# ndoll1998/lightgrad

Measured on AMD Instinct MI355X. Metric: mnist_mlp_train_steps_per_sec_batch1024_per_gpu, higher is better.
Workload: dtype f32; 1 GPU; mnist_mlp_784x512x10_bias_batch1024_mse_adabelief_lr1e-3 (fwd+bwd+allreduce+optimizer); batch_per_gpu=1024, global_batch=1024, parallelism=dp1, optimizer_kernel=fused, input_requires_grad=True, dispatch=hipGraph replay (python tape captured once; 13 consecutive steps per graph), steps_per_graph=13, device=AMD Instinct (gfx950), compute_units=256, clock_mhz=2400

## Files before the change

### lightgrad_amd/csrc/gemm.hip

```cpp
#include "common.h"
#include "gelu_common.h"
#include "adam_common.h"
#include "tail_jobs.h"
#include "mse_finalize.h"
#include "head_fwd_body.h"
#include <cstdlib>
#include <cstring>
#include <type_traits>

namespace lg {

typedef float f32x16 __attribute__((ext_vector_type(16)));
typedef unsigned int u32x4 __attribute__((ext_vector_type(4)));
typedef float f32x4 __attribute__((ext_vector_type(4)));

#ifndef LG_SMALL_PD
#define LG_SMALL_PD 2
#endif
constexpr int kSmallTilePrefetch = LG_SMALL_PD;
#ifndef LG_WAVE_PRIVATE_PD
#define LG_WAVE_PRIVATE_PD 1
#endif
constexpr int kWavePrivatePrefetch = LG_WAVE_PRIVATE_PD;

struct FastDiv {
    uint32_t m, s;
    __device__ __forceinline__ int div(int n) const { return int((uint64_t(uint32_t(n)) * m) >> s); }
};
static FastDiv make_fastdiv(int64_t d) {
    if (d < 1) d = 1;
    uint32_t l = 0;
    while ((int64_t(1) << l) < d) ++l;
    FastDiv f;
    f.m = uint32_t((uint64_t(1) << (31 + l)) / uint64_t(d) + 1);
    f.s = 31 + l;
    return f;
}

struct GemmArgs {
    const float* A;
    const float* B;
    float*       C;
    int64_t M, N, K;
    int64_t lda, ldb, ldc;
    int64_t sA, sB, sC;
    int64_t sA2, sB2, sC2;
    int     batch_inner;
    int     tiles_m, tiles_n;
    int     nwg;
    int     accumulate;
    const float* bias;
    const float* addend;
    int64_t      ldadd;
    int     group_m;
    int     k_slices;
    int64_t k_per_slice;
    float*  W;
    int*    tickets;
    float*  rowsum;
    int     rowsum_accumulate;
    FastDiv div_per_batch, div_slices, div_gspan, div_group, div_last_group, div_batch_inner;
    int     k_tail;
    short   relu_a, relu_b;
    int     act;
    float*  aux;
    int     multi;
    int64_t boff[3], coff[3], biasoff[3];
    int     seg_k, seg_steps;
    int64_t seg_jump[2];
    const AdamPlan* adam_c;
    const AdamPlan* adam_r;
#ifdef LG_GEMM_TIMELINE
    unsigned long long* tl;
#endif
};

#ifdef LG_GEMM_TIMELINE
#define LG_TL(slot) do { if (g.tl && threadIdx.x == 0) g.tl[size_t(blockIdx.x) * 8 + (slot)] = wall_clock64(); } while (0)
#else
#define LG_TL(slot) do { } while (0)
#endif

__device__ __forceinline__ int xcd_remap(int bid, int nwg) {
    const int q = nwg >> 3, r = nwg & 7;
    const int xcd = bid & 7, pos = bid >> 3;
    const int base = xcd < r ? xcd * (q + 1) : r * (q + 1) + (xcd - r) * q;
    return base + pos;
}

template <int BM, int BN> constexpr bool kHasExtras = BM * BN < 256 * 256;
template <int BM, int BN, int KG = 1> constexpr bool kCanSplitK = kHasExtras<BM, BN> && KG == 1;
template <int BM, int BN, int KG = 1> constexpr bool kCanAdam = BM * BN <= 128 * 128 && KG == 1;

#ifdef LG_GEMM_GATHER_STAGING
template <int BM, int BN, bool XKC> constexpr bool kGatherStaging = !XKC && BM * BN == 256 * 256;
#else
template <int BM, int BN, bool XKC> constexpr bool kGatherStaging = false;
#endif
template <int BM, int BN, int WM, int WN, int KG> constexpr bool kWavePrivateTile = KG > 1 && WM * WN == 1 && BM == 32 && BN == 32;
template <int BM, int BN, int BK, bool AKC, bool BKC, int KG>
constexpr int gemm_lds_floats() {
    constexpr int BKS = BK * KG;
    constexpr bool ALK = AKC || kGatherStaging<BM, BN, AKC>, BLK = BKC || kGatherStaging<BM, BN, BKC>;
    return 2 * ((ALK ? BM * (BKS + 4) : BKS * BM) + (BLK ? BN * (BKS + 4) : BKS * BN));
}

template <int BM, int BN, int BK, int WM, int WN, bool AKC, bool BKC, bool VA, bool VB, int PD, int KG = 1, int XT = 0, bool WP = false>
__global__ void __launch_bounds__(WM * WN * KG * 64) sgemm_mfma(GemmArgs g) {
#define LG_TILE_OWNS_LDS 1
#define LG_TILE_BID blockIdx.x
#define LG_TILE_WAVE_PRIVATE WP
#include "gemm_tile_body.inc"
#undef LG_TILE_WAVE_PRIVATE
#undef LG_TILE_OWNS_LDS
#undef LG_TILE_BID
}

struct HeadChain {
    HeadFwd h;
    int*    tickets;
    int     stride;
    int     per_row;
    int*    status;
};
static const HeadChain*& pending_chain() { static const HeadChain* p = nullptr; return p; }
constexpr int kChainTicketBase = 16384, kChainTicketStride = 32, kChainRowBlocks = 64;
template <int OMAX, int PD>
__global__ void __launch_bounds__(256) sgemm_bias_head_fwd(GemmArgs g, HeadChain c) {
    constexpr int BM = 64, BN = 32, BK = 32, WM = 2, WN = 1, KG = 2, XT = 0;
    constexpr bool AKC = true, BKC = true, VA = true, VB = true;
    __shared__ __attribute__((aligned(16))) float lds[gemm_lds_floats<BM, BN, BK, AKC, BKC, KG>()];
    if (int(blockIdx.x) < g.nwg) {
        int* const signal_tickets = c.tickets;
        const int signal_stride = c.stride, signal_per_row = c.per_row;
#define LG_TILE_OWNS_LDS 0
#define LG_TILE_BID int(blockIdx.x)
#undef LG_TILE_SIGNAL
#define LG_TILE_SIGNAL 1
#include "gemm_tile_body.inc"
#undef LG_TILE_SIGNAL
#undef LG_TILE_BID
#undef LG_TILE_OWNS_LDS
    } else {
        const HeadFwd& a = c.h;
        const int tid = threadIdx.x, lane = tid & 63, wave = tid >> 6;
        const int wn = a.outs * a.hidden;
        for (int i = tid * 4; i < wn; i += 1024) *reinterpret_cast<float4*>(lds + i) = *reinterpret_cast<const float4*>(a.w + i);
        const int64_t row0 = int64_t(int(blockIdx.x) - g.nwg) * 4;
        int* const ticket = c.tickets + int(row0 / BM) * c.stride;
        const int64_t block_rows = a.rows - (row0 / BM) * BM < BM ? a.rows - (row0 / BM) * BM : BM;
        const int readers = int((block_rows + 3) / 4);
        int* const flag = ticket + 16;
        int* const done = ticket + 17;
        __shared__ int seen;
        if (tid == 0) {
            int ok = 1;
            const unsigned long long t0 = wall_clock64();
            while (__hip_atomic_load(flag, __ATOMIC_RELAXED, __HIP_MEMORY_SCOPE_AGENT) == 0) {
                __builtin_amdgcn_s_sleep(2);
                if (wall_clock64() - t0 > 200000000ull) {
                    __hip_atomic_fetch_or(c.status, LG_STATUS_HANDOFF_TIMEOUT, __ATOMIC_RELAXED, __HIP_MEMORY_SCOPE_SYSTEM);
                    ok = 0;
                    break;
                }
            }
            seen = ok;
        }
        __syncthreads();
        __builtin_amdgcn_fence(__ATOMIC_ACQUIRE, "wavefront");
        const int64_t row = row0 + wave;
        if (row < a.rows) head_fwd_row<OMAX, true>(a, lds, row, lane);
        if (tid == 0 && seen) {
            if (__hip_atomic_fetch_add(done, 1, __ATOMIC_RELAXED, __HIP_MEMORY_SCOPE_AGENT) == readers - 1) {
                __hip_atomic_store(done, 0, __ATOMIC_RELAXED, __HIP_MEMORY_SCOPE_AGENT);
                __hip_atomic_store(flag, 0, __ATOMIC_RELAXED, __HIP_MEMORY_SCOPE_AGENT);
            }
        }
    }
}

template <int PD, bool SECOND_BKC = false>
__global__ void __launch_bounds__(256) sgemm_pair_wgrad_xgrad(GemmArgs first, GemmArgs second) {
    constexpr int L1 = gemm_lds_floats<64, 64, 32, false, false, 1>(), L2 = gemm_lds_floats<64, 64, 32, true, SECOND_BKC, 1>();
    __shared__ __attribute__((aligned(16))) float lds[L1 > L2 ? L1 : L2];
    constexpr int BM = 64, BN = 64, BK = 32, WM = 2, WN = 2, KG = 1, XT = 0;
    constexpr bool VA = true, VB = true;
#define LG_TILE_OWNS_LDS 0
    if (int(blockIdx.x) < first.nwg) {
        constexpr bool AKC = false, BKC = false;
        const GemmArgs& g = first;
#define LG_TILE_BID int(blockIdx.x)
#include "gemm_tile_body.inc"
#undef LG_TILE_BID
    } else {
        constexpr bool AKC = true, BKC = SECOND_BKC;
        const GemmArgs& g = second;
#define LG_TILE_BID (int(blockIdx.x) - first.nwg)
#include "gemm_tile_body.inc"
#undef LG_TILE_BID
    }
#undef LG_TILE_OWNS_LDS
}

int lg_mse_finalize_job(const float* row_loss, int64_t rows, float inv_n, float* loss);
struct PairFirsts { GemmArgs w[2]; };
struct LossJob {
    const float* row_loss;
    float*       loss;
    int64_t      rows;
    float        inv_n;
};
template <int PD>
__global__ void __launch_bounds__(256) sgemm_triple_wgrad2_xgrad(PairFirsts firsts, GemmArgs second, LossJob job) {
    constexpr int L1 = gemm_lds_floats<64, 64, 32, false, false, 1>(), L2 = gemm_lds_floats<64, 64, 32, true, false, 1>();
    __shared__ __attribute__((aligned(16))) float lds[L1 > L2 ? L1 : L2];
    constexpr int BM = 64, BN = 64, BK = 32, WM = 2, WN = 2, KG = 1, XT = 0;
    constexpr bool VA = true, VB = true;
#define LG_TILE_OWNS_LDS 0
    const int n0w = firsts.w[0].nwg, n1w = firsts.w[1].nwg;
    if (int(blockIdx.x) < n0w + n1w) {
        constexpr bool AKC = false, BKC = false;
        const int which = int(blockIdx.x) >= n0w ? 1 : 0;
        const GemmArgs g = firsts.w[which];
#define LG_TILE_BID (int(blockIdx.x) - (which ? n0w : 0))
#include "gemm_tile_body.inc"
#undef LG_TILE_BID
    } else if (int(blockIdx.x) < n0w + n1w + second.nwg) {
        constexpr bool AKC = true, BKC = false;
        const GemmArgs& g = second;
#define LG_TILE_BID (int(blockIdx.x) - n0w - n1w)
#include "gemm_tile_body.inc"
#undef LG_TILE_BID
    } else {
        finalize_loss(job.row_loss, job.rows, job.inv_n, job.loss, lds);
    }
#undef LG_TILE_OWNS_LDS
}

constexpr int kGroupMax = 14;
struct GroupProduct {
    const float* A;
    const float* B;
    float*       C;
    float*       W;
    int*         tickets;
    float*       rowsum;
    int64_t      M, N, K, lda, ldb, ldc, k_per_slice;
    int          tiles_m, tiles_n, nwg, accumulate, group_m, k_slices, rowsum_accumulate, k_tail;
    FastDiv      div_per_batch, div_slices, div_gspan, div_group, div_last_group, div_batch_inner;
};
static GroupProduct pack_product(const GemmArgs& g) {
    return GroupProduct{g.A, g.B, g.C, g.W, g.tickets, g.rowsum, g.M, g.N, g.K, g.lda, g.ldb, g.ldc, g.k_per_slice,
                        g.tiles_m, g.tiles_n, g.nwg, g.accumulate, g.group_m, g.k_slices, g.rowsum_accumulate, g.k_tail,
                        g.div_per_batch, g.div_slices, g.div_gspan, g.div_group, g.div_last_group, g.div_batch_inner};
}
__device__ __forceinline__ GemmArgs unpack_product(const GroupProduct& p) {
    GemmArgs g{};
    g.A = p.A; g.B = p.B; g.C = p.C; g.W = p.W; g.tickets = p.tickets; g.rowsum = p.rowsum;
    g.M = p.M; g.N = p.N; g.K = p.K; g.lda = p.lda; g.ldb = p.ldb; g.ldc = p.ldc; g.k_per_slice = p.k_per_slice;
    g.tiles_m = p.tiles_m; g.tiles_n = p.tiles_n; g.nwg = p.nwg; g.accumulate = p.accumulate; g.group_m = p.group_m;
    g.k_slices = p.k_slices; g.rowsum_accumulate = p.rowsum_accumulate; g.k_tail = p.k_tail;
    g.div_per_batch = p.div_per_batch; g.div_slices = p.div_slices; g.div_gspan = p.div_gspan; g.div_group = p.div_group;
    g.div_last_group = p.div_last_group; g.div_batch_inner = p.div_batch_inner;
    g.batch_inner = 1;
    return g;
}

struct GemmGroup {
    GroupProduct p[kGroupMax];
    int      first[kGroupMax + 1];
    int      count;
    const float* cs_in;
    float*       cs_out;
    int64_t      cs_rows, cs_cols, cs_ld;
    int          cs_accumulate, cs_wgs;
    int          tail_wgs;
    TailGroup    tail;
};

static_assert(sizeof(GemmGroup) <= 4096, "the group travels as kernel arguments");

template <int PD>
__global__ void __launch_bounds__(256) sgemm_group_wgrad(GemmGroup grp) {
    __shared__ __attribute__((aligned(16))) float lds[gemm_lds_floats<64, 64, 32, false, false, 1>()];
    constexpr int BM = 64, BN = 64, BK = 32, WM = 2, WN = 2, KG = 1, XT = 0;
    constexpr bool VA = true, VB = true, AKC = false, BKC = false;
    if (int(blockIdx.x) < grp.cs_wgs) {
        const int q = threadIdx.x >> 6, cl = threadIdx.x & 63;
        const int64_t col = int64_t(blockIdx.x) * 64 + cl;
        const bool live = col < grp.cs_cols;
        const float* in = grp.cs_in + (live ? col : 0);
        float acc[8] = {0.f, 0.f, 0.f, 0.f, 0.f, 0.f, 0.f, 0.f};
        int64_t r = q;
        for (; r + 28 < grp.cs_rows; r += 32) {
#pragma unroll
            for (int e = 0; e < 8; ++e) acc[e] += in[(r + 4 * e) * grp.cs_ld];
        }
        for (; r < grp.cs_rows; r += 4) acc[0] += in[r * grp.cs_ld];
        lds[threadIdx.x] = ((acc[0] + acc[1]) + (acc[2] + acc[3])) + ((acc[4] + acc[5]) + (acc[6] + acc[7]));
        __syncthreads();
        if (q == 0 && live) {
            const float v = (lds[cl] + lds[64 + cl]) + (lds[128 + cl] + lds[192 + cl]);
            grp.cs_out[col] = grp.cs_accumulate ? grp.cs_out[col] + v : v;
        }
        return;
    }
    const int bid = int(blockIdx.x) - grp.cs_wgs;
    if (bid >= grp.first[grp.count]) {
        tail_group_body(grp.tail, bid - grp.first[grp.count]);
        return;
    }
    int which = 0;
    while (which + 1 < grp.count && bid >= grp.first[which + 1]) ++which;
    const GemmArgs g = unpack_product(grp.p[which]);
// ... 9 lines not shown
template <int BM, int BN, int BK, int WM, int WN, bool AKC, bool BKC, int KG>
static bool launch_layout(const GemmArgs& g, bool va, bool vb) {
    dim3 grid(g.nwg), block(WM * WN * KG * 64);
    hipStream_t s = rt().stream;
    constexpr int PD = (BM * BN <= 64 * 64) ? kSmallTilePrefetch : 2;
    static_assert(BM * BN < 256 * 256 || PD <= 2, "a third K-tile in flight does not fit the 256x256 tile's 128 registers: ring registers would spill while their loads are in flight");
    if constexpr (kWavePrivateTile<BM, BN, WM, WN, KG> && AKC && BKC) {
        static const char* kloop_env = getenv("LG_GEMM_KLOOP");
        if (va && vb && !(kloop_env && strcmp(kloop_env, "coop") == 0)) {
            constexpr int WPD = kWavePrivatePrefetch;
            if (g.multi) hipLaunchKernelGGL((sgemm_mfma<BM, BN, BK, WM, WN, true, true, true, true, WPD, KG, 1, true>), grid, block, 0, s, g);
            else         hipLaunchKernelGGL((sgemm_mfma<BM, BN, BK, WM, WN, true, true, true, true, WPD, KG, 0, true>), grid, block, 0, s, g);
            return true;
        }
    }
    if constexpr (kHasExtras<BM, BN>) {
        if constexpr (AKC && BKC)  { if (g.multi) { hipLaunchKernelGGL((sgemm_mfma<BM, BN, BK, WM, WN, AKC, BKC, true, true, PD, KG, 1>), grid, block, 0, s, g); return false; } }
        if constexpr (AKC && !BKC) { if (g.seg_k) { hipLaunchKernelGGL((sgemm_mfma<BM, BN, BK, WM, WN, AKC, BKC, true, true, PD, KG, 2>), grid, block, 0, s, g); return false; } }
    }
    if constexpr (!kHasExtras<BM, BN>) {
        hipLaunchKernelGGL((sgemm_mfma<BM, BN, BK, WM, WN, AKC, BKC, true, true, PD, KG>), grid, block, 0, s, g);
        return false;
    }
    if (va && vb)  hipLaunchKernelGGL((sgemm_mfma<BM, BN, BK, WM, WN, AKC, BKC, true, true, PD, KG>), grid, block, 0, s, g);
    else if (va)   hipLaunchKernelGGL((sgemm_mfma<BM, BN, BK, WM, WN, AKC, BKC, true, false, 1, KG>), grid, block, 0, s, g);
    else if (vb)   hipLaunchKernelGGL((sgemm_mfma<BM, BN, BK, WM, WN, AKC, BKC, false, true, 1, KG>), grid, block, 0, s, g);
    else           hipLaunchKernelGGL((sgemm_mfma<BM, BN, BK, WM, WN, AKC, BKC, false, false, 1, KG>), grid, block, 0, s, g);
    return false;
}

#ifdef LG_GEMM_TIMELINE
static void lg_debug_timeline_state(unsigned long long* buf, int nwg, int slices, int tiles);
#endif
struct PairState {
    int      active = 0;
    int      count = 0;
    bool     second_bkc = false;
    GemmArgs args[3];
    bool     is_s[3] = {false, false, false};
    int64_t  batch[3] = {1, 1, 1};
    int64_t  tiles = 0;
    LossJob  job{};
};
static PairState& pair_state() { static PairState p; return p; }

static void pair_launch_single(const GemmArgs& g, bool is_s) {
    dim3 grid(g.nwg), block(256);
    constexpr int PD = kSmallTilePrefetch;
    if (!is_s) hipLaunchKernelGGL((sgemm_mfma<64, 64, 32, 2, 2, false, false, true, true, PD, 1>), grid, block, 0, rt().stream, g);
    else if (pair_state().second_bkc) hipLaunchKernelGGL((sgemm_mfma<64, 64, 32, 2, 2, true, true, true, true, PD, 1>), grid, block, 0, rt().stream, g);
    else           hipLaunchKernelGGL((sgemm_mfma<64, 64, 32, 2, 2, true, false, true, true, PD, 1>), grid, block, 0, rt().stream, g);
}

static int pair_retune(GemmArgs& g, int64_t others_nwg) {
    const int64_t tiles = int64_t(g.tiles_m) * g.tiles_n;
    static const char* pair_slices_env = getenv("LG_GEMM_PAIR_SLICES");
    if (pair_slices_env || g.nwg != tiles * g.k_slices || g.seg_k || tiles >= 256 || g.K < 128) return LG_OK;
    constexpr int BK = 32, BM = 64, BN = 64;
    const double cus = rt().compute_units > 0 ? rt().compute_units : 256;
    const int64_t k_tiles = (g.K + BK - 1) / BK;
    int64_t best_sl = g.k_slices;
    double best = 1e30;
    for (int64_t sl = 1; sl <= 64 && (sl == 1 || sl * 2 <= k_tiles); ++sl) {
        const double per_cu = double(tiles * sl + others_nwg) / cus;
        const double c = per_cu > 1.0 ? double(int64_t(per_cu + 0.999)) : 1.0;
        const double cost = double((k_tiles + sl - 1) / sl) * (c <= 1.0 ? 0.68 : 0.43 * c + 0.17) + (sl > 1 ? 1.8 + 0.85 * double(sl) : 0.0);
        if (cost < best) { best = cost; best_sl = sl; }
    }
    int64_t k_per_slice = ((g.K + best_sl - 1) / best_sl + BK - 1) / BK * BK;
    best_sl = (g.K + k_per_slice - 1) / k_per_slice;
    if (best_sl == g.k_slices) return LG_OK;
    if (g.W) { const int rc = lg_free(g.W); g.W = nullptr; if (rc != LG_OK) return rc; }
    g.k_per_slice = k_per_slice;
    g.k_slices = int(best_sl);
    g.nwg = int(tiles * best_sl);
    g.div_slices = make_fastdiv(best_sl);
    if (best_sl > 1) {
        const int rc = lg_malloc(reinterpret_cast<void**>(&g.W), size_t(tiles * best_sl) * BM * BN * sizeof(float));
        if (rc != LG_OK) return rc;
    }
    return LG_OK;
}

static int pair_flush(bool keep_collecting) {
    PairState& P = pair_state();
    int rc = LG_OK;
    bool job_done = false;
    if (P.count == 3) {
        rc = pair_retune(P.args[1], int64_t(P.args[0].nwg) + P.args[2].nwg);
        if (rc != LG_OK) { P.count = 0; return rc; }
        PairFirsts firsts;
        firsts.w[0] = P.args[0];
        firsts.w[1] = P.args[1];
        const int spare = P.job.loss ? 1 : 0;
        hipLaunchKernelGGL((sgemm_triple_wgrad2_xgrad<kSmallTilePrefetch>), dim3(P.args[0].nwg + P.args[1].nwg + P.args[2].nwg + spare), dim3(256), 0,
                           rt().stream, firsts, P.args[2], P.job);
        job_done = true;
    } else if (P.count == 2 && P.is_s[1]) {
        rc = pair_retune(P.args[0], P.args[1].nwg);
        if (rc != LG_OK) { P.count = 0; return rc; }
#ifdef LG_GEMM_TIMELINE
        if (P.args[0].tl) {
            (void)hipMemsetAsync(P.args[0].tl, 0, size_t(P.args[0].nwg + P.args[1].nwg) * 64, rt().stream);
            lg_debug_timeline_state(P.args[0].tl, P.args[0].nwg + P.args[1].nwg, P.args[0].k_slices * 100 + P.args[1].k_slices, P.args[0].nwg);
        }
#endif
        if (P.second_bkc)
            hipLaunchKernelGGL((sgemm_pair_wgrad_xgrad<kSmallTilePrefetch, true>), dim3(P.args[0].nwg + P.args[1].nwg), dim3(256), 0, rt().stream,
                               P.args[0], P.args[1]);
        else
            hipLaunchKernelGGL((sgemm_pair_wgrad_xgrad<kSmallTilePrefetch, false>), dim3(P.args[0].nwg + P.args[1].nwg), dim3(256), 0, rt().stream,
                               P.args[0], P.args[1]);
    } else {
        for (int i = 0; i < P.count; ++i) pair_launch_single(P.args[i], P.is_s[i]);
    }
    for (int i = 0; i < P.count; ++i)
        if (P.args[i].W) { const int r = lg_free(P.args[i].W); if (r != LG_OK) rc = r; }
    P.count = 0;
    P.tiles = 0;
    if (job_done) P.job = LossJob{};
    if (!keep_collecting && P.active) P.active = 2;
    return rc;
}

struct WriteSpan { uintptr_t lo, hi; };
static WriteSpan product_c_span(const GemmArgs& g, int64_t batch) {
    const int64_t outer = batch / g.batch_inner;
    int64_t lo = 0, hi = (g.M - 1) * g.ldc + g.N;
    const int64_t reach[2] = {(outer - 1) * g.sC, int64_t(g.batch_inner - 1) * g.sC2};
    for (int64_t r : reach) { if (r < 0) lo += r; else hi += r; }
    const uintptr_t base = reinterpret_cast<uintptr_t>(g.C);
    return WriteSpan{base + uintptr_t(lo * 4), base + uintptr_t(hi * 4)};
}
static bool spans_meet(WriteSpan a, WriteSpan b) { return a.lo < b.hi && b.lo < a.hi; }
static bool products_write_alike(const GemmArgs& a, int64_t batch_a, const GemmArgs& b, int64_t batch_b) {
    const WriteSpan none{0, 0};
    const WriteSpan ca = product_c_span(a, batch_a), cb = product_c_span(b, batch_b);
    const WriteSpan ra = a.rowsum ? WriteSpan{reinterpret_cast<uintptr_t>(a.rowsum), reinterpret_cast<uintptr_t>(a.rowsum + a.M)} : none;
    const WriteSpan rb = b.rowsum ? WriteSpan{reinterpret_cast<uintptr_t>(b.rowsum), reinterpret_cast<uintptr_t>(b.rowsum + b.M)} : none;
    return spans_meet(ca, cb) || spans_meet(ca, rb) || spans_meet(ra, cb) || spans_meet(ra, rb);
}

static bool pair_try_defer(GemmArgs& g, bool akc, bool bkc, bool va, bool vb, int64_t batch) {
    PairState& P = pair_state();
    if (P.active != 1) return false;
    const int slot = P.count;
    for (int i = 0; i < slot; ++i)
        if (products_write_alike(P.args[i], P.batch[i], g, batch)) return false;
    const bool f_form = !akc && !bkc, s_form = akc;
    bool fits = slot < 3 && va && vb && batch >= 1;
    if (slot == 0)      fits = fits && f_form;
    else if (slot == 1) fits = fits && !P.is_s[0] && (f_form || s_form);
    else                fits = fits && !P.is_s[1] && s_form && !bkc && batch == 1 && !g.relu_a && !g.relu_b;
    if (slot == 1 && f_form) fits = fits && batch == 1 && P.args[0].nwg == int64_t(P.args[0].tiles_m) * P.args[0].tiles_n * P.args[0].k_slices;
    const int64_t tiles = int64_t(g.tiles_m) * g.tiles_n * batch;
    if (!fits || P.tiles + tiles > rt().n_tickets) return false;
    g.tickets = rt().tickets + P.tiles;
    P.tiles += tiles;
    if (s_form) P.second_bkc = bkc;
    P.is_s[slot] = s_form;
    P.args[slot] = g;
    P.batch[slot] = batch;
    P.count = slot + 1;
    return true;
}

constexpr int kGroupTiles = 1024;
struct GroupState {
    int       active = 0;
    int       count = 0;
    int64_t   tiles = 0;
    GemmArgs  queued[kGroupMax];
    GemmGroup grp;
};
static GroupState& group_state() { static GroupState s; return s; }

static int group_flush() {
    GroupState& G = group_state();
    if (G.count == 0) {
        if (G.grp.cs_wgs > 0) {
            const int64_t shape[2] = {G.grp.cs_rows, G.grp.cs_cols}, strides[2] = {G.grp.cs_ld, 1};
            G.grp.cs_wgs = 0;
            return lg_reduce_acc(LG_RED_SUM, 2, shape, G.grp.cs_in, strides, 1u, G.grp.cs_out, G.grp.cs_accumulate);
        }
        return LG_OK;
    }
    int rc = LG_OK;
    if (G.count == 1 && G.grp.cs_wgs == 0) {
        pair_launch_single(G.queued[0], 0);
    } else {
        GemmArgs sorted[kGroupMax];
        int n = 0;
        for (int pass = 0; pass < 2; ++pass)
            for (int i = 0; i < G.count; ++i)
                if ((G.queued[i].nwg > 256) == (pass == 1)) sorted[n++] = G.queued[i];
// ... 568 lines not shown
```

### lightgrad_amd/csrc/gemm_tile_body.inc

```
#ifndef LG_TILE_SIGNAL
#define LG_TILE_SIGNAL 0
#endif
#ifndef LG_TILE_WAVE_PRIVATE
#define LG_TILE_WAVE_PRIVATE false
#endif
    constexpr bool WPK = LG_TILE_WAVE_PRIVATE;
    static_assert(!WPK || (KG > 1 && WM * WN == 1 && BM == 32 && BN == 32 && AKC && BKC && VA && VB && XT != 2 && !LG_TILE_SIGNAL), "wave-private K loop: one wave per K-group, NT form");
    constexpr int NT = WM * WN * KG * 64;
    constexpr int NTS = WPK ? 64 : NT;
    constexpr int BKS = WPK ? BK : BK * KG;
    constexpr int TM = BM / WM / 32, TN = BN / WN / 32;
    static_assert(TM >= 1 && TN >= 1 && BK % 16 == 0 && (KG == 1 || KG == 2 || KG == 4), "tile config");
    constexpr bool AG = kGatherStaging<BM, BN, AKC>, BG = kGatherStaging<BM, BN, BKC>;
    static_assert((!AG || VA) && (!BG || VB), "gather staging replaces the float4 form");
    constexpr bool ALK = AKC || AG, BLK = BKC || BG;
    constexpr int A_PITCH = ALK ? BKS + 4 : BM;
    constexpr int B_PITCH = BLK ? BKS + 4 : BN;
    constexpr int A_TILE = ALK ? BM * A_PITCH : BKS * A_PITCH;
    constexpr int B_TILE = BLK ? BN * B_PITCH : BKS * B_PITCH;
    constexpr int A_ELEMS = BM * BKS / NTS, B_ELEMS = BN * BKS / NTS;
    static_assert(A_ELEMS % 4 == 0 && B_ELEMS % 4 == 0, "staging must divide into float4");

    static_assert(WPK || 2 * (A_TILE + B_TILE) == gemm_lds_floats<BM, BN, BK, AKC, BKC, KG>(), "LDS size");
    static_assert(!(AG || BG) || TM * TN > 1, "gather staging: the multi-accumulator loop only");
#if LG_TILE_OWNS_LDS
    __shared__ __attribute__((aligned(16))) float lds[gemm_lds_floats<BM, BN, BK, AKC, BKC, KG>()];
#endif
    constexpr int BUF = A_TILE + B_TILE;

    const int tid = threadIdx.x;
    const int lane = tid & 63, wave = tid >> 6;
    const int kg = WPK ? __builtin_amdgcn_readfirstlane(wave) : wave / (WM * WN), wl = wave % (WM * WN);
    const int wm = wl / WN, wn = wl % WN;
    const int kofs = WPK ? 0 : kg * BK;
    const int stid = WPK ? lane : tid;
    float* const ldsw = WPK ? lds + kg * BUF : lds;
    const int r = lane & 31, h = lane >> 5;
    LG_TL(0);

    const int id = xcd_remap(LG_TILE_BID, g.nwg);
    const int per_batch = g.tiles_m * g.tiles_n;
    const int bs = g.div_per_batch.div(id);
    const int batch = g.div_slices.div(bs), slice = bs - batch * g.k_slices;
    const int t = id - bs * per_batch;
    const int GROUP_M = g.group_m;
    const int gspan = GROUP_M * g.tiles_n;
    const int group = g.div_gspan.div(t);
    const int first_m = group * GROUP_M, in_group = t - group * gspan;
    const bool last_group = g.tiles_m - first_m < GROUP_M;
    const int gsize = last_group ? g.tiles_m - first_m : GROUP_M;
    const int tn = last_group ? g.div_last_group.div(in_group) : g.div_group.div(in_group);
    const int tm = first_m + (in_group - tn * gsize);
    const int64_t m0 = int64_t(tm) * BM, n0 = int64_t(tn) * BN;
    const int b_outer = g.div_batch_inner.div(batch), b_inner = batch - b_outer * g.batch_inner;
    const float* __restrict__ A = g.A + int64_t(b_outer) * g.sA + int64_t(b_inner) * g.sA2;
    const float* Bp = g.B + int64_t(b_outer) * g.sB + int64_t(b_inner) * g.sB2;
    float* Cp = g.C + int64_t(b_outer) * g.sC + int64_t(b_inner) * g.sC2;
    const float* biasp = g.bias;
    if constexpr (XT == 1) {
        {
            Bp += batch == 0 ? g.boff[0] : batch == 1 ? g.boff[1] : g.boff[2];
            Cp += batch == 0 ? g.coff[0] : batch == 1 ? g.coff[1] : g.coff[2];
            if (biasp) biasp += batch == 0 ? g.biasoff[0] : batch == 1 ? g.biasoff[1] : g.biasoff[2];
        }
    }
    const float* __restrict__ B = Bp;
    float* __restrict__ C = Cp;
    const int64_t ldc = g.ldc;
    const int accumulate = g.accumulate;
    const float* __restrict__ bias = biasp;
    const int64_t k_begin = int64_t(slice) * g.k_per_slice;
    const int64_t k_end = (k_begin + g.k_per_slice < g.K) ? k_begin + g.k_per_slice : g.K;
    const bool has_virtual = kHasExtras<BM, BN> && g.rowsum != nullptr && n0 <= g.N && g.N < n0 + BN;

    using StageA = std::conditional_t<VA, f32x4, float>;
    using StageB = std::conditional_t<VB, f32x4, float>;
    constexpr int A_CHUNKS = VA ? A_ELEMS / 4 : A_ELEMS, B_CHUNKS = VB ? B_ELEMS / 4 : B_ELEMS;
    constexpr int NL = (kGatherStaging<BM, BN, AKC> ? 4 : 1) * A_CHUNKS + (kGatherStaging<BM, BN, BKC> ? 4 : 1) * B_CHUNKS;
    static_assert((PD - 1) * NL + NL <= 63, "vmcnt is a 6-bit counter");
    StageA ra_ring[PD][A_CHUNKS];
    StageB rb_ring[PD][B_CHUNKS];
    [[maybe_unused]] float ga_ring[PD][AG ? A_CHUNKS : 1][4];
    [[maybe_unused]] float gb_ring[PD][BG ? B_CHUNKS : 1][4];

    constexpr unsigned OOB = 0x80000000u;
    constexpr int A_W = VA ? 4 : 1, B_W = VB ? 4 : 1;
    constexpr int A_DIV = AG ? BM : (AKC ? BKS : BM) / A_W, B_DIV = BG ? BN : (BKC ? BKS : BN) / B_W;
    static_assert(NTS % A_DIV == 0 && NTS % B_DIV == 0, "a thread's chunks must differ by whole rows");
    constexpr int A_STEP = NTS / A_DIV, B_STEP = NTS / B_DIV;
    const int a_q = stid / A_DIV, a_r = AG ? stid % A_DIV : (stid % A_DIV) * A_W;
    const int b_q = stid / B_DIV, b_r = BG ? stid % B_DIV : (stid % B_DIV) * B_W;
    auto kcA = [&](int i) { return AG ? 4 * (a_q + i * A_STEP) : (AKC ? a_r : a_q + i * A_STEP); };
    auto kcB = [&](int i) { return BG ? 4 * (b_q + i * B_STEP) : (BKC ? b_r : b_q + i * B_STEP); };
    const int a_lds0 = AG ? a_r * A_PITCH + 4 * a_q : a_q * A_PITCH + a_r, b_lds0 = BG ? b_r * B_PITCH + 4 * b_q : b_q * B_PITCH + b_r;
    constexpr int A_LDS_STEP = AG ? 4 * A_STEP : A_STEP * A_PITCH, B_LDS_STEP = BG ? 4 * B_STEP : B_STEP * B_PITCH;
    unsigned offA[A_CHUNKS], offB[B_CHUNKS];
    unsigned virt_mask = 0;
    int krem_ring[PD];
#pragma unroll
    for (int i = 0; i < A_CHUNKS; ++i) {
        const int row = AKC ? a_q + i * A_STEP : a_r, kk = kcA(i);
        const unsigned bytes = AKC ? (unsigned(row) * unsigned(g.lda) + unsigned(kk)) * 4u : (unsigned(kk) * unsigned(g.lda) + unsigned(row)) * 4u;
        offA[i] = (m0 + row < g.M) ? bytes : OOB;
    }
#pragma unroll
    for (int i = 0; i < B_CHUNKS; ++i) {
        const int col = BKC ? b_q + i * B_STEP : b_r, kk = kcB(i);
        const unsigned bytes = BKC ? (unsigned(col) * unsigned(g.ldb) + unsigned(kk)) * 4u : (unsigned(kk) * unsigned(g.ldb) + unsigned(col)) * 4u;
        offB[i] = (n0 + col < g.N) ? bytes : OOB;
        if (has_virtual && n0 + col == g.N) virt_mask |= 1u << i;
    }
    const float* const Atile0 = AKC ? A + m0 * g.lda : A + m0;
    const float* const Btile0 = BKC ? B + n0 * g.ldb : B + n0;

    auto descriptor = [](const float* base) {
        const unsigned long long p = reinterpret_cast<unsigned long long>(base);
        u32x4 d;
        d[0] = unsigned(p); d[1] = unsigned(p >> 32) & 0xffffu; d[2] = OOB; d[3] = 0x00020000u;
        return d;
    };
    constexpr int KSTEP = BK * KG;
    int64_t wk_begin = k_begin, wk_len = k_end - k_begin;
    if constexpr (WPK) {
        wk_begin = k_begin + kg * BK;
        wk_len = wk_len - kg * BK;
        wk_len = wk_len < 0 ? 0 : wk_len;
    }
    const float* nextA = AKC ? Atile0 + wk_begin : Atile0 + wk_begin * g.lda;
    const float* nextB = BKC ? Btile0 + wk_begin : Btile0 + wk_begin * g.ldb;
    const int64_t stepA = AKC ? int64_t(KSTEP) : int64_t(KSTEP) * g.lda, stepB = BKC ? int64_t(KSTEP) : int64_t(KSTEP) * g.ldb;
    [[maybe_unused]] const unsigned gatherA = unsigned(g.lda) * 4u, gatherB = unsigned(g.ldb) * 4u;
    const int nkt = int((wk_len + KSTEP - 1) / KSTEP);
    const int last_left = int(wk_len) - (nkt - 1) * KSTEP;
    const int last_krem = last_left < BKS ? last_left : BKS;
    int requested = 0;
    int seg_left = 0, seg_idx = 0;
    if constexpr (XT == 2) seg_left = g.seg_steps;
    auto load_tile = [&](int slot) {
        const int krem = requested == nkt - 1 ? last_krem : BKS;
        ++requested;
        krem_ring[slot] = krem;
        const u32x4 da = descriptor(nextA);
        const u32x4 db = descriptor(nextB);
        nextA += stepA;
        nextB += stepB;
        if constexpr (XT == 2) {
            if (--seg_left == 0) {
                nextB += seg_idx ? g.seg_jump[1] : g.seg_jump[0];
                seg_idx = 1;
                seg_left = g.seg_steps;
            }
        }
#pragma unroll
        for (int i = 0; i < A_CHUNKS; ++i) {
            if constexpr (AG) {
                if (krem == BKS) {
#pragma unroll
                    for (int e = 0; e < 4; ++e)
                        asm volatile("buffer_load_dword %0, %1, %2, %3 offen" : "=v"(ga_ring[slot][i][e]) : "v"(offA[i]), "s"(da), "s"(unsigned(e) * gatherA));
                } else {
#pragma unroll
                    for (int e = 0; e < 4; ++e) {
                        const unsigned off = kcA(i) + e < krem ? offA[i] : OOB;
                        asm volatile("buffer_load_dword %0, %1, %2, %3 offen" : "=v"(ga_ring[slot][i][e]) : "v"(off), "s"(da), "s"(unsigned(e) * gatherA));
                    }
                }
            } else {
                const unsigned off = kcA(i) < krem ? offA[i] : OOB;
                if constexpr (VA) asm volatile("buffer_load_dwordx4 %0, %1, %2, 0 offen" : "=v"(ra_ring[slot][i]) : "v"(off), "s"(da));
                else              asm volatile("buffer_load_dword %0, %1, %2, 0 offen" : "=v"(ra_ring[slot][i]) : "v"(off), "s"(da));
            }
        }
#pragma unroll
        for (int i = 0; i < B_CHUNKS; ++i) {
            if constexpr (BG) {
                if (krem == BKS) {
#pragma unroll
                    for (int e = 0; e < 4; ++e)
                        asm volatile("buffer_load_dword %0, %1, %2, %3 offen" : "=v"(gb_ring[slot][i][e]) : "v"(offB[i]), "s"(db), "s"(unsigned(e) * gatherB));
                } else {
#pragma unroll
                    for (int e = 0; e < 4; ++e) {
                        const unsigned off = kcB(i) + e < krem ? offB[i] : OOB;
                        asm volatile("buffer_load_dword %0, %1, %2, %3 offen" : "=v"(gb_ring[slot][i][e]) : "v"(off), "s"(db), "s"(unsigned(e) * gatherB));
                    }
                }
            } else {
                const unsigned off = kcB(i) < krem ? offB[i] : OOB;
                if constexpr (VB) asm volatile("buffer_load_dwordx4 %0, %1, %2, 0 offen" : "=v"(rb_ring[slot][i]) : "v"(off), "s"(db));
                else              asm volatile("buffer_load_dword %0, %1, %2, 0 offen" : "=v"(rb_ring[slot][i]) : "v"(off), "s"(db));
            }
        }
    };
    auto wait_tile = [&](int slot, int younger) {
        if (PD >= 3 && younger >= 2)      asm volatile("s_waitcnt vmcnt(%0)" :: "n"(PD >= 3 ? 2 * NL : 0) : "memory");
        else if (PD >= 2 && younger == 1) asm volatile("s_waitcnt vmcnt(%0)" :: "n"(PD >= 2 ? NL : 0) : "memory");
// ... 68 lines not shown
                if constexpr (VB) {
                    if constexpr (BKC) {
                        if (virt) {
                            const int kr = krem_ring[slot] - kcB(i);
                            rb_ring[slot][i] = f32x4{kr > 0 ? 1.f : 0.f, kr > 1 ? 1.f : 0.f, kr > 2 ? 1.f : 0.f, kr > 3 ? 1.f : 0.f};
                        }
                    }
                    else               { if (virt) rb_ring[slot][i] = f32x4{one, 0.f, 0.f, 0.f}; }
                } else {
                    if (virt) rb_ring[slot][i] = one;
                }
            }
        }
#pragma unroll
        for (int i = 0; i < B_CHUNKS; ++i) {
            if constexpr (BG)      *reinterpret_cast<f32x4*>(b + b_lds0 + i * B_LDS_STEP) = f32x4{gb_ring[slot][i][0], gb_ring[slot][i][1], gb_ring[slot][i][2], gb_ring[slot][i][3]};
            else if constexpr (VB) *reinterpret_cast<f32x4*>(b + b_lds0 + i * B_LDS_STEP) = rb_ring[slot][i];
            else                   b[b_lds0 + i * B_LDS_STEP] = rb_ring[slot][i];
        }
    };

    f32x16 acc[TM][TN];
    [[maybe_unused]] float bias_ahead[TN];
    if constexpr (kHasExtras<BM, BN>) {
#pragma unroll
        for (int j = 0; j < TN; ++j) {
            const int64_t col = n0 + (wn * TN + j) * 32 + r;
            bias_ahead[j] = (bias && col < g.N) ? bias[col] : 0.f;
        }
    }
#pragma unroll
    for (int i = 0; i < TM; ++i)
#pragma unroll
        for (int j = 0; j < TN; ++j)
#pragma unroll
            for (int e = 0; e < 16; ++e) acc[i][j][e] = 0.f;

    auto compute_tile = [&](int buf, int kb_begin, int kb_end) {
        const float* a = lds + buf * BUF + (ALK ? (wm * TM * 32 + r) * A_PITCH + 4 * h + kofs : (4 * h + kofs) * A_PITCH + wm * TM * 32 + r);
        const float* b = lds + buf * BUF + A_TILE + (BLK ? (wn * TN * 32 + r) * B_PITCH + 4 * h + kofs : (4 * h + kofs) * B_PITCH + wn * TN * 32 + r);
#pragma unroll
        for (int kb = kb_begin; kb < kb_end; kb += 8) {
            float fa[TM][4], fb[TN][4];
#pragma unroll
            for (int i = 0; i < TM; ++i) {
                if constexpr (ALK) {
                    const float4 v = *reinterpret_cast<const float4*>(a + i * 32 * A_PITCH + kb);
                    fa[i][0] = v.x; fa[i][1] = v.y; fa[i][2] = v.z; fa[i][3] = v.w;
                } else {
#pragma unroll
                    for (int s = 0; s < 4; ++s) fa[i][s] = a[(kb + s) * A_PITCH + i * 32];
                }
            }
#pragma unroll
            for (int j = 0; j < TN; ++j) {
                if constexpr (BLK) {
                    const float4 v = *reinterpret_cast<const float4*>(b + j * 32 * B_PITCH + kb);
                    fb[j][0] = v.x; fb[j][1] = v.y; fb[j][2] = v.z; fb[j][3] = v.w;
                } else {
#pragma unroll
                    for (int s = 0; s < 4; ++s) fb[j][s] = b[(kb + s) * B_PITCH + j * 32];
                }
            }
#pragma unroll
            for (int s = 0; s < 4; ++s)
#pragma unroll
                for (int i = 0; i < TM; ++i)
#pragma unroll
                    for (int j = 0; j < TN; ++j)
                        acc[i][j] = __builtin_amdgcn_mfma_f32_32x32x2f32(fa[i][s], fb[j][s], acc[i][j], 0, 0, 0);
        }
    };

#pragma unroll
    for (int u = 0; u < PD; ++u)
        if (u < nkt) load_tile(u);
    if constexpr (!WPK) {
        const int younger = nkt - 1 < PD - 1 ? nkt - 1 : PD - 1;
        wait_tile(0, younger);
        store_tile(0, 0);
        __syncthreads();
    }
    LG_TL(1);
    if constexpr (WPK) {
        static_assert(BK == 16, "one K-step is two k-blocks of 8");
        float fa[2][4], fb[2][4];
        auto read_half = [&](int half, int set) {
            const float4 va = *reinterpret_cast<const float4*>(ldsw + r * A_PITCH + 4 * h + half * 8);
            const float4 vb = *reinterpret_cast<const float4*>(ldsw + A_TILE + r * B_PITCH + 4 * h + half * 8);
            fa[set][0] = va.x; fa[set][1] = va.y; fa[set][2] = va.z; fa[set][3] = va.w;
            fb[set][0] = vb.x; fb[set][1] = vb.y; fb[set][2] = vb.z; fb[set][3] = vb.w;
        };
        auto mfma_part = [&](int set, int e0, int e1) {
#pragma unroll
            for (int e = e0; e < e1; ++e)
                acc[0][0] = __builtin_amdgcn_mfma_f32_32x32x2f32(fa[set][e], fb[set][e], acc[0][0], 0, 0, 0);
        };
        auto advance = [&](int t, int slot) {
            const int younger = (nkt < t + PD ? nkt : t + PD) - (t + 1);
            wait_tile(slot, younger);
            store_tile(0, slot);
            if (t + PD < nkt) load_tile(slot);
        };
        if (nkt > 0) {
            advance(0, 0);
            read_half(0, 0);
        }
        for (int kt0 = 0; kt0 < nkt; kt0 += PD) {
#pragma unroll
            for (int u = 0; u < PD; ++u) {
                const int kt = kt0 + u;
                if (kt < nkt) {
                    read_half(1, 1);
                    mfma_part(0, 0, 4);
                    __builtin_amdgcn_sched_barrier(0);
                    if (kt + 1 < nkt) advance(kt + 1, (u + 1) % PD);
                    __builtin_amdgcn_sched_barrier(0);
                    mfma_part(1, 0, 1);
                    __builtin_amdgcn_sched_barrier(0);
                    if (kt + 1 < nkt) read_half(0, 0);
                    mfma_part(1, 1, 4);
                }
            }
        }
    } else if constexpr (TM * TN == 1) {
        constexpr int HG = BK / 16;
        float fa[2][HG][4], fb[2][HG][4];
        auto read_half = [&](int buf, int half, int slot) {
            const float* a = lds + buf * BUF + (AKC ? (wm * 32 + r) * A_PITCH + 4 * h + kofs : (4 * h + kofs) * A_PITCH + wm * 32 + r);
            const float* b = lds + buf * BUF + A_TILE + (BKC ? (wn * 32 + r) * B_PITCH + 4 * h + kofs : (4 * h + kofs) * B_PITCH + wn * 32 + r);
#pragma unroll
            for (int q = 0; q < HG; ++q) {
                const int kb = half * (BK / 2) + q * 8;
                if constexpr (AKC) {
                    const float4 v = *reinterpret_cast<const float4*>(a + kb);
                    fa[slot][q][0] = v.x; fa[slot][q][1] = v.y; fa[slot][q][2] = v.z; fa[slot][q][3] = v.w;
                } else {
#pragma unroll
                    for (int e = 0; e < 4; ++e) fa[slot][q][e] = a[(kb + e) * A_PITCH];
                }
                if constexpr (BKC) {
                    const float4 v = *reinterpret_cast<const float4*>(b + kb);
                    fb[slot][q][0] = v.x; fb[slot][q][1] = v.y; fb[slot][q][2] = v.z; fb[slot][q][3] = v.w;
                } else {
#pragma unroll
                    for (int e = 0; e < 4; ++e) fb[slot][q][e] = b[(kb + e) * B_PITCH];
                }
            }
        };
        auto mfma_part = [&](int slot, int q0, int q1) {
#pragma unroll
            for (int q = q0; q < q1; ++q)
#pragma unroll
                for (int e = 0; e < 4; ++e)
                    acc[0][0] = __builtin_amdgcn_mfma_f32_32x32x2f32(fa[slot][q][e], fb[slot][q][e], acc[0][0], 0, 0, 0);
        };
        auto mfma_half = [&](int slot) { mfma_part(slot, 0, HG); };
        constexpr int HQ = HG > 1 ? HG / 2 : HG;
        read_half(0, 0, 0);
        for (int kt0 = 0; kt0 < nkt; kt0 += PD) {
#pragma unroll
            for (int u = 0; u < PD; ++u) {
                const int kt = kt0 + u;
                if (kt < nkt) {
                    const int cur = kt & 1;
                    if (PD == 1 && kt + 1 < nkt) load_tile(0);
                    read_half(cur, 1, 1);
                    mfma_part(0, 0, HQ);
                    __builtin_amdgcn_sched_barrier(0);
                    if (kt + 1 < nkt) {
                        int younger = nkt - (kt + 2);
                        if (younger > PD - 2) younger = PD - 2;
                        wait_tile((u + 1) % PD, PD == 1 ? 0 : (younger < 0 ? 0 : younger));
                        store_tile(cur ^ 1, (u + 1) % PD);
                    }
                    if (PD > 1 && kt + PD < nkt) load_tile(u);
                    __builtin_amdgcn_sched_barrier(0);
                    mfma_part(0, HQ, HG);
                    __syncthreads();
                    if (kt + 1 < nkt) read_half(cur ^ 1, 0, 0);
                    mfma_half(1);
                }
            }
        }
    } else {
        for (int kt0 = 0; kt0 < nkt; kt0 += PD) {
    #pragma unroll
            for (int u = 0; u < PD; ++u) {
                const int kt = kt0 + u;
                if (kt < nkt) {
                    const int cur = kt & 1;
                    if (PD == 1 && kt + 1 < nkt) load_tile(0);
                    compute_tile(cur, 0, BK / 2);
                    if (kt + 1 < nkt) {
                        int younger = nkt - (kt + 2);
                        if (younger > PD - 2) younger = PD - 2;
                        wait_tile((u + 1) % PD, PD == 1 ? 0 : (younger < 0 ? 0 : younger));
                        store_tile(cur ^ 1, (u + 1) % PD);
                    }
                    if (PD > 1 && kt + PD < nkt) load_tile(u);
                    compute_tile(cur, BK / 2, BK);
                    __syncthreads();
                }
            }
        }
    }

    LG_TL(2);
    if constexpr (KG > 1) {
        constexpr int GROUP_FLOATS = WM * WN * TM * TN * 16 * 64;
        static_assert(WPK || (KG - 1) * GROUP_FLOATS <= 2 * (A_TILE + B_TILE), "the K-group exchange must fit the staging buffers");
        static_assert(!WPK || KG * BUF + (KG - 1) * GROUP_FLOATS <= gemm_lds_floats<BM, BN, BK, AKC, BKC, KG>(), "staging regions + exchange");
        float* x = lds + (WPK ? KG * BUF : 0) + (wl * TM * TN * 16) * 64 + lane;
        if (kg >= 1) {
#pragma unroll
            for (int i = 0; i < TM; ++i)
#pragma unroll
                for (int j = 0; j < TN; ++j)
#pragma unroll
                    for (int e = 0; e < 16; ++e) x[(kg - 1) * GROUP_FLOATS + ((i * TN + j) * 16 + e) * 64] = acc[i][j][e];
        }
        __syncthreads();
        if (kg >= 1) return;
#pragma unroll
        for (int gq = 0; gq < KG - 1; ++gq)
#pragma unroll
            for (int i = 0; i < TM; ++i)
#pragma unroll
                for (int j = 0; j < TN; ++j)
#pragma unroll
                    for (int e = 0; e < 16; ++e) acc[i][j][e] += x[gq * GROUP_FLOATS + ((i * TN + j) * 16 + e) * 64];
    }
    [[maybe_unused]] AdamScalars adam_cs_c, adam_cs_r;
    [[maybe_unused]] int64_t adam_done_c = 0, adam_done_r = 0;
    if constexpr (kCanAdam<BM, BN, KG>) {
        if (g.adam_c) adam_cs_c = adam_plan_scalars(g.adam_c, adam_done_c);
        if (g.adam_r) adam_cs_r = adam_plan_scalars(g.adam_r, adam_done_r);
    }
    if constexpr (kCanSplitK<BM, BN, KG>) if (g.k_slices > 1) {
        constexpr int SC1 = 16;
        constexpr int TILE_BYTES = BM * BN * 4;
        char* slab0 = reinterpret_cast<char*>(g.W) + (int64_t(batch) * g.k_slices * per_batch + t) * int64_t(TILE_BYTES);
        const int64_t slice_stride = int64_t(per_batch) * TILE_BYTES;
        {
            const auto mine = __builtin_amdgcn_make_buffer_rsrc(slab0 + slice * slice_stride, 0, TILE_BYTES, 0x00020000);
#pragma unroll
            for (int i = 0; i < TM; ++i)
#pragma unroll
// ... 174 lines not shown
```

Before: 21220 steps/s.

## Add wave-private quadrant K-loop for dX GEMM and raise wgrad wave priority

```diff
diff --git a/lightgrad_amd/csrc/gemm.hip b/lightgrad_amd/csrc/gemm.hip
--- a/lightgrad_amd/csrc/gemm.hip
+++ b/lightgrad_amd/csrc/gemm.hip
@@ -22,6 +22,11 @@
 #define LG_WAVE_PRIVATE_PD 1
 #endif
 constexpr int kWavePrivatePrefetch = LG_WAVE_PRIVATE_PD;
+#ifndef LG_QUADRANT_PD
+#define LG_QUADRANT_PD 1
+#endif
+constexpr int kQuadrantPrefetch = LG_QUADRANT_PD;
+constexpr int kQuadrantStageFloats = 32 * (32 + 4) + 32 * 32;
 
 struct FastDiv {
     uint32_t m, s;
@@ -179,24 +184,31 @@
     }
 }
 
-template <int PD, bool SECOND_BKC = false>
+template <int PDK, bool SECOND_BKC = false, bool WPRIO = false, bool DXWP = false>
 __global__ void __launch_bounds__(256) sgemm_pair_wgrad_xgrad(GemmArgs first, GemmArgs second) {
     constexpr int L1 = gemm_lds_floats<64, 64, 32, false, false, 1>(), L2 = gemm_lds_floats<64, 64, 32, true, SECOND_BKC, 1>();
     __shared__ __attribute__((aligned(16))) float lds[L1 > L2 ? L1 : L2];
+    static_assert(!DXWP || (!SECOND_BKC && 4 * kQuadrantStageFloats <= (L1 > L2 ? L1 : L2)), "four single-buffered wave regions within the cooperative loop's LDS");
     constexpr int BM = 64, BN = 64, BK = 32, WM = 2, WN = 2, KG = 1, XT = 0;
     constexpr bool VA = true, VB = true;
 #define LG_TILE_OWNS_LDS 0
     if (int(blockIdx.x) < first.nwg) {
+        if constexpr (WPRIO) __builtin_amdgcn_s_setprio(1);
         constexpr bool AKC = false, BKC = false;
+        constexpr int PD = PDK;
         const GemmArgs& g = first;
 #define LG_TILE_BID int(blockIdx.x)
 #include "gemm_tile_body.inc"
 #undef LG_TILE_BID
     } else {
         constexpr bool AKC = true, BKC = SECOND_BKC;
+        constexpr int PD = DXWP ? kQuadrantPrefetch : PDK;
         const GemmArgs& g = second;
 #define LG_TILE_BID (int(blockIdx.x) - first.nwg)
+#undef LG_TILE_WAVE_PRIVATE
+#define LG_TILE_WAVE_PRIVATE DXWP
 #include "gemm_tile_body.inc"
+#undef LG_TILE_WAVE_PRIVATE
 #undef LG_TILE_BID
     }
 #undef LG_TILE_OWNS_LDS
@@ -210,16 +222,19 @@
     int64_t      rows;
     float        inv_n;
 };
-template <int PD>
+template <int PDK, bool WPRIO = false, bool DXWP = false>
 __global__ void __launch_bounds__(256) sgemm_triple_wgrad2_xgrad(PairFirsts firsts, GemmArgs second, LossJob job) {
     constexpr int L1 = gemm_lds_floats<64, 64, 32, false, false, 1>(), L2 = gemm_lds_floats<64, 64, 32, true, false, 1>();
     __shared__ __attribute__((aligned(16))) float lds[L1 > L2 ? L1 : L2];
+    static_assert(!DXWP || 4 * kQuadrantStageFloats <= (L1 > L2 ? L1 : L2), "four single-buffered wave regions within the cooperative loop's LDS");
     constexpr int BM = 64, BN = 64, BK = 32, WM = 2, WN = 2, KG = 1, XT = 0;
     constexpr bool VA = true, VB = true;
 #define LG_TILE_OWNS_LDS 0
     const int n0w = firsts.w[0].nwg, n1w = firsts.w[1].nwg;
     if (int(blockIdx.x) < n0w + n1w) {
+        if constexpr (WPRIO) __builtin_amdgcn_s_setprio(1);
         constexpr bool AKC = false, BKC = false;
+        constexpr int PD = PDK;
         const int which = int(blockIdx.x) >= n0w ? 1 : 0;
         const GemmArgs g = firsts.w[which];
 #define LG_TILE_BID (int(blockIdx.x) - (which ? n0w : 0))
@@ -227,9 +242,13 @@
 #undef LG_TILE_BID
     } else if (int(blockIdx.x) < n0w + n1w + second.nwg) {
         constexpr bool AKC = true, BKC = false;
+        constexpr int PD = DXWP ? kQuadrantPrefetch : PDK;
         const GemmArgs& g = second;
 #define LG_TILE_BID (int(blockIdx.x) - n0w - n1w)
+#undef LG_TILE_WAVE_PRIVATE
+#define LG_TILE_WAVE_PRIVATE DXWP
 #include "gemm_tile_body.inc"
+#undef LG_TILE_WAVE_PRIVATE
 #undef LG_TILE_BID
     } else {
         finalize_loss(job.row_loss, job.rows, job.inv_n, job.loss, lds);
@@ -405,6 +424,15 @@
     return LG_OK;
 }
 
+static bool pair_wgrad_prio() {
+    static const char* prio_env = getenv("LG_GEMM_WGRAD_PRIO");
+    return !(prio_env && atoi(prio_env) == 0);
+}
+static bool pair_dx_wave_private(const GemmArgs& second, bool second_bkc) {
+    static const char* kloop_env = getenv("LG_GEMM_PAIR_KLOOP");
+    return !(kloop_env && strcmp(kloop_env, "coop") == 0) && !second_bkc && second.k_slices == 1;
+}
+
 static int pair_flush(bool keep_collecting) {
     PairState& P = pair_state();
     int rc = LG_OK;
@@ -416,8 +444,20 @@
         firsts.w[0] = P.args[0];
         firsts.w[1] = P.args[1];
         const int spare = P.job.loss ? 1 : 0;
-        hipLaunchKernelGGL((sgemm_triple_wgrad2_xgrad<kSmallTilePrefetch>), dim3(P.args[0].nwg + P.args[1].nwg + P.args[2].nwg + spare), dim3(256), 0,
-                           rt().stream, firsts, P.args[2], P.job);
+#ifdef LG_GEMM_TIMELINE
+        if (P.args[0].tl) {
+            const int all = P.args[0].nwg + P.args[1].nwg + P.args[2].nwg + spare;
+            (void)hipMemsetAsync(P.args[0].tl, 0, size_t(all) * 64, rt().stream);
+            lg_debug_timeline_state(P.args[0].tl, all, (P.args[0].k_slices * 100 + P.args[1].k_slices) * 100 + P.args[2].k_slices, P.args[0].nwg + P.args[1].nwg);
+        }
+#endif
+        const dim3 grid(P.args[0].nwg + P.args[1].nwg + P.args[2].nwg + spare);
+        const bool prio = pair_wgrad_prio(), dxwp = pair_dx_wave_private(P.args[2], false);
+        constexpr int PD = kSmallTilePrefetch;
+        if (prio && dxwp) hipLaunchKernelGGL((sgemm_triple_wgrad2_xgrad<PD, true, true>), grid, dim3(256), 0, rt().stream, firsts, P.args[2], P.job);
+        else if (prio)    hipLaunchKernelGGL((sgemm_triple_wgrad2_xgrad<PD, true, false>), grid, dim3(256), 0, rt().stream, firsts, P.args[2], P.job);
+        else if (dxwp)    hipLaunchKernelGGL((sgemm_triple_wgrad2_xgrad<PD, false, true>), grid, dim3(256), 0, rt().stream, firsts, P.args[2], P.job);
+        else              hipLaunchKernelGGL((sgemm_triple_wgrad2_xgrad<PD, false, false>), grid, dim3(256), 0, rt().stream, firsts, P.args[2], P.job);
         job_done = true;
     } else if (P.count == 2 && P.is_s[1]) {
         rc = pair_retune(P.args[0], P.args[1].nwg);
@@ -428,12 +468,16 @@
             lg_debug_timeline_state(P.args[0].tl, P.args[0].nwg + P.args[1].nwg, P.args[0].k_slices * 100 + P.args[1].k_slices, P.args[0].nwg);
         }
 #endif
-        if (P.second_bkc)
-            hipLaunchKernelGGL((sgemm_pair_wgrad_xgrad<kSmallTilePrefetch, true>), dim3(P.args[0].nwg + P.args[1].nwg), dim3(256), 0, rt().stream,
-                               P.args[0], P.args[1]);
-        else
-            hipLaunchKernelGGL((sgemm_pair_wgrad_xgrad<kSmallTilePrefetch, false>), dim3(P.args[0].nwg + P.args[1].nwg), dim3(256), 0, rt().stream,
-                               P.args[0], P.args[1]);
+        const dim3 grid(P.args[0].nwg + P.args[1].nwg);
+        const bool prio = pair_wgrad_prio(), dxwp = pair_dx_wave_private(P.args[1], P.second_bkc);
+        constexpr int PD = kSmallTilePrefetch;
+        if (P.second_bkc) {
+            if (prio) hipLaunchKernelGGL((sgemm_pair_wgrad_xgrad<PD, true, true, false>), grid, dim3(256), 0, rt().stream, P.args[0], P.args[1]);
+            else      hipLaunchKernelGGL((sgemm_pair_wgrad_xgrad<PD, true, false, false>), grid, dim3(256), 0, rt().stream, P.args[0], P.args[1]);
+        }
+        else if (prio && dxwp) hipLaunchKernelGGL((sgemm_pair_wgrad_xgrad<PD, false, true, true>), grid, dim3(256), 0, rt().stream, P.args[0], P.args[1]);
+        else if (dxwp)         hipLaunchKernelGGL((sgemm_pair_wgrad_xgrad<PD, false, false, true>), grid, dim3(256), 0, rt().stream, P.args[0], P.args[1]);
+        else                   hipLaunchKernelGGL((sgemm_pair_wgrad_xgrad<PD, false, false, false>), grid, dim3(256), 0, rt().stream, P.args[0], P.args[1]);
     } else {
         for (int i = 0; i < P.count; ++i) pair_launch_single(P.args[i], P.is_s[i]);
     }
diff --git a/lightgrad_amd/csrc/gemm_tile_body.inc b/lightgrad_amd/csrc/gemm_tile_body.inc
--- a/lightgrad_amd/csrc/gemm_tile_body.inc
+++ b/lightgrad_amd/csrc/gemm_tile_body.inc
@@ -5,20 +5,24 @@
 #define LG_TILE_WAVE_PRIVATE false
 #endif
     constexpr bool WPK = LG_TILE_WAVE_PRIVATE;
-    static_assert(!WPK || (KG > 1 && WM * WN == 1 && BM == 32 && BN == 32 && AKC && BKC && VA && VB && XT != 2 && !LG_TILE_SIGNAL), "wave-private K loop: one wave per K-group, NT form");
+    constexpr bool WPQ = WPK && KG == 1;
+    static_assert(!WPK || (AKC && VA && VB && XT != 2 && !LG_TILE_SIGNAL), "wave-private K loop: K-contiguous A, float4 staging");
+    static_assert(!WPK || WPQ || (KG > 1 && WM * WN == 1 && BM == 32 && BN == 32 && BKC), "wave-private K loop: one wave per K-group, NT form");
+    static_assert(!WPQ || (BM / WM == 32 && BN / WN == 32 && BK == 32 && !BKC && XT == 0), "wave-private K loop, quadrant form: one accumulator per wave, N-contiguous B");
     constexpr int NT = WM * WN * KG * 64;
     constexpr int NTS = WPK ? 64 : NT;
     constexpr int BKS = WPK ? BK : BK * KG;
+    constexpr int SM = WPQ ? BM / WM : BM, SN = WPQ ? BN / WN : BN;
     constexpr int TM = BM / WM / 32, TN = BN / WN / 32;
     static_assert(TM >= 1 && TN >= 1 && BK % 16 == 0 && (KG == 1 || KG == 2 || KG == 4), "tile config");
     constexpr bool AG = kGatherStaging<BM, BN, AKC>, BG = kGatherStaging<BM, BN, BKC>;
     static_assert((!AG || VA) && (!BG || VB), "gather staging replaces the float4 form");
     constexpr bool ALK = AKC || AG, BLK = BKC || BG;
-    constexpr int A_PITCH = ALK ? BKS + 4 : BM;
-    constexpr int B_PITCH = BLK ? BKS + 4 : BN;
-    constexpr int A_TILE = ALK ? BM * A_PITCH : BKS * A_PITCH;
-    constexpr int B_TILE = BLK ? BN * B_PITCH : BKS * B_PITCH;
-    constexpr int A_ELEMS = BM * BKS / NTS, B_ELEMS = BN * BKS / NTS;
+    constexpr int A_PITCH = ALK ? BKS + 4 : SM;
+    constexpr int B_PITCH = BLK ? BKS + 4 : SN;
+    constexpr int A_TILE = ALK ? SM * A_PITCH : BKS * A_PITCH;
+    constexpr int B_TILE = BLK ? SN * B_PITCH : BKS * B_PITCH;
+    constexpr int A_ELEMS = SM * BKS / NTS, B_ELEMS = SN * BKS / NTS;
     static_assert(A_ELEMS % 4 == 0 && B_ELEMS % 4 == 0, "staging must divide into float4");
 
     static_assert(WPK || 2 * (A_TILE + B_TILE) == gemm_lds_floats<BM, BN, BK, AKC, BKC, KG>(), "LDS size");
@@ -30,11 +34,12 @@
 
     const int tid = threadIdx.x;
     const int lane = tid & 63, wave = tid >> 6;
-    const int kg = WPK ? __builtin_amdgcn_readfirstlane(wave) : wave / (WM * WN), wl = wave % (WM * WN);
+    const int swave = WPK ? __builtin_amdgcn_readfirstlane(wave) : wave;
+    const int kg = WPQ ? 0 : (WPK ? swave : wave / (WM * WN)), wl = WPQ ? swave : wave % (WM * WN);
     const int wm = wl / WN, wn = wl % WN;
     const int kofs = WPK ? 0 : kg * BK;
     const int stid = WPK ? lane : tid;
-    float* const ldsw = WPK ? lds + kg * BUF : lds;
+    float* const ldsw = WPK ? lds + swave * BUF : lds;
     const int r = lane & 31, h = lane >> 5;
     LG_TL(0);
 
@@ -52,6 +57,7 @@
     const int tn = last_group ? g.div_last_group.div(in_group) : g.div_group.div(in_group);
     const int tm = first_m + (in_group - tn * gsize);
     const int64_t m0 = int64_t(tm) * BM, n0 = int64_t(tn) * BN;
+    const int64_t m0s = WPQ ? m0 + wm * SM : m0, n0s = WPQ ? n0 + wn * SN : n0;
     const int b_outer = g.div_batch_inner.div(batch), b_inner = batch - b_outer * g.batch_inner;
     const float* __restrict__ A = g.A + int64_t(b_outer) * g.sA + int64_t(b_inner) * g.sA2;
     const float* Bp = g.B + int64_t(b_outer) * g.sB + int64_t(b_inner) * g.sB2;
@@ -85,7 +91,7 @@
 
     constexpr unsigned OOB = 0x80000000u;
     constexpr int A_W = VA ? 4 : 1, B_W = VB ? 4 : 1;
-    constexpr int A_DIV = AG ? BM : (AKC ? BKS : BM) / A_W, B_DIV = BG ? BN : (BKC ? BKS : BN) / B_W;
+    constexpr int A_DIV = AG ? BM : (AKC ? BKS : SM) / A_W, B_DIV = BG ? BN : (BKC ? BKS : SN) / B_W;
     static_assert(NTS % A_DIV == 0 && NTS % B_DIV == 0, "a thread's chunks must differ by whole rows");
     constexpr int A_STEP = NTS / A_DIV, B_STEP = NTS / B_DIV;
     const int a_q = stid / A_DIV, a_r = AG ? stid % A_DIV : (stid % A_DIV) * A_W;
@@ -101,17 +107,17 @@
     for (int i = 0; i < A_CHUNKS; ++i) {
         const int row = AKC ? a_q + i * A_STEP : a_r, kk = kcA(i);
         const unsigned bytes = AKC ? (unsigned(row) * unsigned(g.lda) + unsigned(kk)) * 4u : (unsigned(kk) * unsigned(g.lda) + unsigned(row)) * 4u;
-        offA[i] = (m0 + row < g.M) ? bytes : OOB;
+        offA[i] = (m0s + row < g.M) ? bytes : OOB;
     }
 #pragma unroll
     for (int i = 0; i < B_CHUNKS; ++i) {
         const int col = BKC ? b_q + i * B_STEP : b_r, kk = kcB(i);
         const unsigned bytes = BKC ? (unsigned(col) * unsigned(g.ldb) + unsigned(kk)) * 4u : (unsigned(kk) * unsigned(g.ldb) + unsigned(col)) * 4u;
-        offB[i] = (n0 + col < g.N) ? bytes : OOB;
-        if (has_virtual && n0 + col == g.N) virt_mask |= 1u << i;
-    }
-    const float* const Atile0 = AKC ? A + m0 * g.lda : A + m0;
-    const float* const Btile0 = BKC ? B + n0 * g.ldb : B + n0;
+        offB[i] = (n0s + col < g.N) ? bytes : OOB;
+        if (has_virtual && n0s + col == g.N) virt_mask |= 1u << i;
+    }
+    const float* const Atile0 = AKC ? A + m0s * g.lda : A + m0s;
+    const float* const Btile0 = BKC ? B + n0s * g.ldb : B + n0s;
 
     auto descriptor = [](const float* base) {
         const unsigned long long p = reinterpret_cast<unsigned long long>(base);
@@ -346,7 +352,7 @@
         __syncthreads();
     }
     LG_TL(1);
-    if constexpr (WPK) {
+    if constexpr (WPK && !WPQ) {
         static_assert(BK == 16, "one K-step is two k-blocks of 8");
         float fa[2][4], fb[2][4];
         auto read_half = [&](int half, int set) {
@@ -387,6 +393,57 @@
                 }
             }
         }
+    } else if constexpr (WPQ) {
+        constexpr int HG = BK / 16;
+        float fa[2][HG][4], fb[2][HG][4];
+        const float* const fra = ldsw + r * A_PITCH + 4 * h;
+        const float* const frb = ldsw + A_TILE + 4 * h * B_PITCH + r;
+        auto read_half = [&](int half, int set) {
+#pragma unroll
+            for (int q = 0; q < HG; ++q) {
+                const int kb = half * (BK / 2) + q * 8;
+                const float4 v = *reinterpret_cast<const float4*>(fra + kb);
+                fa[set][q][0] = v.x; fa[set][q][1] = v.y; fa[set][q][2] = v.z; fa[set][q][3] = v.w;
+#pragma unroll
+                for (int e = 0; e < 4; ++e) fb[set][q][e] = frb[(kb + e) * B_PITCH];
+            }
+        };
+        auto mfma_part = [&](int set, int i0, int i1) {
+#pragma unroll
+            for (int i = i0; i < i1; ++i)
+                acc[0][0] = __builtin_amdgcn_mfma_f32_32x32x2f32(fa[set][i / 4][i % 4], fb[set][i / 4][i % 4], acc[0][0], 0, 0, 0);
+        };
+        auto advance = [&](int t, int slot) {
+            const int younger = (nkt < t + PD ? nkt : t + PD) - (t + 1);
+            wait_tile(slot, younger);
+            store_tile(0, slot);
+            if (t + PD < nkt) load_tile(slot);
+        };
+        if (nkt > 0) {
+            advance(0, 0);
+            read_half(0, 0);
+        }
+        for (int kt0 = 0; kt0 < nkt; kt0 += PD) {
+#pragma unroll
+            for (int u = 0; u < PD; ++u) {
+                const int kt = kt0 + u;
+                if (kt < nkt) {
+#ifdef LG_GEMM_TIMELINE
+                    if (kt == nkt / 2) LG_TL(7);
+#endif
+                    read_half(1, 1);
+                    mfma_part(0, 0, 4);
+                    __builtin_amdgcn_sched_barrier(0);
+                    if (kt + 1 < nkt) advance(kt + 1, (u + 1) % PD);
+                    __builtin_amdgcn_sched_barrier(0);
+                    mfma_part(0, 4, HG * 4);
+                    mfma_part(1, 0, 1);
+                    __builtin_amdgcn_sched_barrier(0);
+                    if (kt + 1 < nkt) read_half(0, 0);
+                    mfma_part(1, 1, HG * 4);
+                }
+            }
+        }
     } else if constexpr (TM * TN == 1) {
         constexpr int HG = BK / 16;
         float fa[2][HG][4], fb[2][HG][4];
@@ -428,6 +485,9 @@
                 const int kt = kt0 + u;
                 if (kt < nkt) {
                     const int cur = kt & 1;
+#ifdef LG_GEMM_TIMELINE
+                    if (kt == nkt / 2) LG_TL(7);
+#endif
                     if (PD == 1 && kt + 1 < nkt) load_tile(0);
                     read_half(cur, 1, 1);
                     mfma_part(0, 0, HQ);
```

New measurement: 20780 steps/s. 0.98x the previous value.
